# 0xC0000054/avif-format

Measured on NVIDIA H100. Metric: Gpixels/s, higher is better.
Workload: dtype f32

## Files before the change

### avif-format_b200/csrc/avifgpu_api.cu

```cuda
#include "../../include/avifgpu.h"

#include "batch_plan.h"
#include "curve_tables.h"
#include "host_params.h"
#include "kernel_params.h"

#include <cuda_runtime.h>

#include <algorithm>
#include <atomic>
#include <condition_variable>
#include <cstdio>
#include <cstdlib>
#include <cstring>
#include <mutex>
#include <new>
#include <string>
#include <thread>
#include <vector>


namespace avifgpu
{
namespace
{
    thread_local int g_launchFailure = 0;
}

int ReportLaunchFailure(int cudaErrorCode)
{
    g_launchFailure = cudaErrorCode;
    return AVIFGPU_ERR_CUDA;
}

static int TakeLaunchFailure()
{
    const int code = g_launchFailure;
    g_launchFailure = 0;
    return code;
}

int LaunchEncode(const EncodeParams& params, int hostDepth, void* stream)
{
    const EncodeFamily family = EncodeFamilyOf(params, hostDepth);
    const Interior inner = EncodeBlockInterior(family, params, hostDepth);
    if (inner.width == 0)
    {
        return LaunchEncodeGeneric(params, hostDepth, stream);
    }
    cudaError_t e;
    switch (family)
    {
    case EncodeFamily::RgbF32Interleaved: e = LaunchEncodeRgbF32Interleaved(params, inner, stream); break;
    case EncodeFamily::Gray16Lut: e = LaunchEncodeGray16Lut(params, inner, stream); break;
    case EncodeFamily::GrayInt: e = LaunchEncodeGrayInt(params, hostDepth, inner, stream); break;
    case EncodeFamily::RgbInt: e = LaunchEncodeRgbInt(params, hostDepth, inner, stream); break;
    case EncodeFamily::GrayF32: e = LaunchEncodeGrayF32(params, inner, stream); break;
    default: e = LaunchEncodeRgbF32Planar(family, params, inner, stream); break;
    }
    return CompleteEncode(e, params, hostDepth, inner.width, inner.rows, stream);
}

// ... 282 lines not shown
    void FirstUseEncode(const avifgpu_encode_desc& d, int64_t pixels, bool capturing, EncodeParams* p)
    {
        if (CurveTable* table = CurveTableFor(d, pixels, false, capturing))
        {
            p->curveTable = table->valid ? &table->view : nullptr;
        }
        p->gray16Lut = Gray16LutFor(d, capturing);
        p->verifiedPremultiply = VerifiedPremultiply(d, capturing);
    }

    void FirstUseDecode(const avifgpu_decode_desc& d, int32_t transfer, bool capturing, DecodeParams* p)
    {
        p->verifiedHlgDivisions = (d.host_depth == 32 && transfer == AVIFGPU_TRANSFER_HLG) ? VerifiedHlgDivisions(capturing) : 0;
        p->verifiedGreenDivision = VerifiedGreenDivision(*p, capturing);
        p->verifiedPqRatio = (d.host_depth == 32 && transfer == AVIFGPU_TRANSFER_PQ && d.colorspace == AVIFGPU_COLORSPACE_YCBCR) ? VerifiedPqRatio(capturing) : 0;
    }

    int Fail(int status, const std::string& message)
    {
        lastError = message;
        return status;
    }

    int LaunchFailed(int status, const char* what, bool capturing = false)
    {
        const int code = TakeLaunchFailure();
        for (const Slot& slot : slots)
        {
            if (slot.stream && !capturing)
            {
                cudaStreamSynchronize(slot.stream);
            }
        }
        cudaGetLastError();
        lastError = std::string(what) + " failed: " + (code != 0 ? cudaGetErrorString(static_cast<cudaError_t>(code)) : avifgpu_status_string(status));
        return status;
    }

    int Cuda(cudaError_t e, const char* what)
    {
        if (e == cudaSuccess)
        {
            return AVIFGPU_OK;
        }
        lastError = std::string(what) + ": " + cudaGetErrorString(e);
        return (e == cudaErrorMemoryAllocation) ? AVIFGPU_ERR_OOM : AVIFGPU_ERR_CUDA;
// ... 170 lines not shown
    }
    avifgpu_context* ctx = new (std::nothrow) avifgpu_context();
    if (ctx == nullptr)
    {
        g_creationError = "out of host memory";
        return AVIFGPU_ERR_OOM;
    }
    ctx->device = device_ordinal;
    ctx->smCount = prop.multiProcessorCount;
    DeviceGuard guard(device_ordinal);
    for (int i = 0; i < kPipelineStreams; ++i)
    {
        avifgpu_context::Slot& slot = ctx->slots[i];
        if (cudaStreamCreateWithFlags(&slot.stream, cudaStreamNonBlocking) != cudaSuccess ||
            cudaEventCreateWithFlags(&slot.sliceDone, cudaEventDisableTiming) != cudaSuccess ||
            cudaEventCreateWithFlags(&slot.rowsConsumed, cudaEventDisableTiming) != cudaSuccess ||
            (i < 2 && cudaEventCreateWithFlags(&ctx->callRowsConsumed[i], cudaEventDisableTiming) != cudaSuccess))
        {
            g_creationError = std::string("stream/event creation failed: ") + cudaGetErrorString(cudaGetLastError());
            avifgpu_destroy(ctx);
            return AVIFGPU_ERR_CUDA;
        }
    }
    *out_ctx = ctx;
    return AVIFGPU_OK;
}

AVIFGPU_EXPORT void avifgpu_destroy(avifgpu_context* ctx)
{
    if (ctx == nullptr)
    {
        return;
    }
    DeviceGuard guard(ctx->device);
    cudaDeviceSynchronize();
    for (int i = 0; i < kPipelineStreams; ++i)
    {
        const avifgpu_context::Slot& slot = ctx->slots[i];
        if (slot.stream) cudaStreamDestroy(slot.stream);
        if (slot.sliceDone) cudaEventDestroy(slot.sliceDone);
        if (slot.rowsConsumed) cudaEventDestroy(slot.rowsConsumed);
        if (i < 2 && ctx->callRowsConsumed[i]) cudaEventDestroy(ctx->callRowsConsumed[i]);
        for (int b = 0; b < kSlotBuffers; ++b)
        {
            if (slot.device[b].ptr) cudaFree(slot.device[b].ptr);
            if (slot.pinned[b].ptr) cudaFreeHost(slot.pinned[b].ptr);
        }
    }
    for (auto& b : ctx->transferScratch)
    {
        if (b.ptr) cudaFree(b.ptr);
    }
    for (CurveTable* t : ctx->curveTables)
    {
        FreeCurveTable(t);
        delete t;
    }
    for (auto& l : ctx->gray16Luts)
    {
        cudaFree(l.device);
    }
    delete ctx;
}

AVIFGPU_EXPORT const char* avifgpu_last_error(const avifgpu_context* ctx)
{
    return ctx ? ctx->lastError.c_str() : g_creationError.c_str();
}

AVIFGPU_EXPORT int64_t avifgpu_launch_count(const avifgpu_context* ctx) { return ctx ? ctx->launches : 0; }

AVIFGPU_EXPORT int avifgpu_synchronize(avifgpu_context* ctx)
{
    if (ctx == nullptr)
    {
// ... 152 lines not shown
    p.rowCount = nrows;
    for (int k = 0; k < AVIFGPU_MAX_PLANES; ++k)
    {
        const PlaneGeometry g = EncodePlaneGeometry(*desc, k);
        if (!g.present)
        {
            continue;
        }
        if (device_dst->data[k] == nullptr)
        {
            return ctx->Fail(AVIFGPU_ERR_BAD_PARAM, "missing destination plane");
        }
        p.plane[k] = static_cast<uint8_t*>(device_dst->data[k]) + static_cast<int64_t>(y0 >> g.ys) * device_dst->stride[k];
        p.planeStride[k] = device_dst->stride[k];
    }
    DeviceGuard guard(ctx->device);
    bool capturing;
    if ((status = QueryCapture(ctx, cuda_stream, &capturing)) != AVIFGPU_OK)
    {
        return status;
    }
    p.smCount = ctx->smCount;
    ctx->FirstUseEncode(*desc, static_cast<int64_t>(desc->width) * nrows, capturing, &p);
    const int launched = LaunchEncode(p, desc->host_depth, cuda_stream);
    if (launched < 0)
    {
        return ctx->LaunchFailed(launched, "encode kernel launch", capturing);
    }
    ctx->launches += launched;
    return AVIFGPU_OK;
}

AVIFGPU_EXPORT int avifgpu_decode_rows_device(avifgpu_context* ctx, const avifgpu_decode_desc* desc,
                                              const avifgpu_planes* device_src, int32_t y0, int32_t nrows, void* device_rows,
                                              int64_t row_stride_bytes, void* cuda_stream)
{
    if (ctx == nullptr)
    {
        return AVIFGPU_ERR_BAD_PARAM;
    }
    avifgpu_decode_desc full;
    desc = WidenDecodeDesc(desc, &full);
    std::string error;
    int32_t transfer;
    int status = ValidateDecodeDesc(desc, &transfer, &error);
    if (status != AVIFGPU_OK)
    {
// ... 102 lines not shown
    bool capturing;
    int status = QueryCapture(ctx, cuda_stream, &capturing);
    if (status != AVIFGPU_OK)
    {
        return status;
    }
    shared.smCount = ctx->smCount;
    ctx->FirstUseEncode(*desc, pixels, capturing, &shared);
    BatchPlan plan;
    PlanEncodeBatch(shared, desc->host_depth, planeMask, images, count, &plan);
    for (const BatchChunk& chunk : plan.chunks)
    {
        const int launched = LaunchEncodeBatchChunk(shared, desc->host_depth, chunk, cuda_stream);
        if (launched < 0)
        {
            return ctx->LaunchFailed(launched, "batched encode kernel launch", capturing);
        }
        ctx->launches += launched;
    }
    for (const int32_t i : plan.fallback)
    {
        EncodeParams p = shared;
        AdoptBatchImage(p, planeMask, images[i]);
        const int launched = LaunchEncode(p, desc->host_depth, cuda_stream);
        if (launched < 0)
        {
            return ctx->LaunchFailed(launched, "encode kernel launch", capturing);
        }
        ctx->launches += launched;
    }
    return AVIFGPU_OK;
}

AVIFGPU_EXPORT int avifgpu_decode_batch_device(avifgpu_context* ctx, const avifgpu_decode_desc* desc, const avifgpu_batch_image* images,
                                               int32_t count, void* cuda_stream)
{
    if (ctx == nullptr)
    {
        return AVIFGPU_ERR_BAD_PARAM;
    }
    if (desc == nullptr || count < 0 || (count > 0 && images == nullptr))
    {
        return ctx->Fail(AVIFGPU_ERR_BAD_PARAM, "NULL description or image array");
    }
    avifgpu_decode_desc full;
    desc = WidenDecodeDesc(desc, &full);
    avifgpu_decode_desc d = *desc;
// ... 664 lines not shown
            (status = ctx->Cuda(cudaEventRecord(slot.rowsConsumed, slot.stream), "cudaEventRecord")) != AVIFGPU_OK) return AbandonCall(ctx, status);
        callSlots[index] = true;
        if (!wait && rowsPinned && begin + sliceRows >= nrows)
        {
            for (int s = 0; s < kPipelineStreams; ++s)
            {
                if (s != index && callSlots[s] &&
                    (status = ctx->Cuda(cudaStreamWaitEvent(slot.stream, ctx->slots[s].rowsConsumed, 0), "cudaStreamWaitEvent")) != AVIFGPU_OK) return AbandonCall(ctx, status);
            }
            if ((status = ctx->Cuda(cudaEventRecord(ctx->callRowsConsumed[ctx->asyncEncodeCalls & 1], slot.stream), "cudaEventRecord")) != AVIFGPU_OK) return AbandonCall(ctx, status);
            recordedCallRows = true;
        }

        if ((status = EnsureDeviceStaging(ctx, slot, out, planes)) != AVIFGPU_OK) return AbandonCall(ctx, status);
        EncodeParams p = base;
        p.rows = slot.device[kRowsBuffer].ptr;
        p.rowStride = deviceRowStride;
        p.rowCount = rows;
        for (int i = 0; i < planes; ++i)
        {
            p.plane[out[i].buffer] = slot.device[out[i].buffer].ptr;
            p.planeStride[out[i].buffer] = out[i].deviceStride;
        }
        const int launched = LaunchEncode(p, desc->host_depth, slot.stream);
        if (launched < 0)
        {
            return AbandonCall(ctx, ctx->LaunchFailed(launched, "encode kernel launch"));
        }
        ctx->launches += launched;

        if ((status = StageOut(ctx, slot, out, planes)) != AVIFGPU_OK || (status = CloseSlice(ctx, slot, ticket)) != AVIFGPU_OK) return AbandonCall(ctx, status);
    }
    status = FinishCall(ctx, previousRows, ticket, wait);
    if (status == AVIFGPU_OK && !wait && recordedCallRows)
    {
        ctx->asyncEncodeCalls += 1;
        ctx->previousCallRowsPending = true;
    }
    return status;
}

static int DecodeRowsHost(avifgpu_context* ctx, const avifgpu_decode_desc* desc, const avifgpu_planes* src, int32_t y0, int32_t nrows,
                          void* host_rows, int64_t row_stride_bytes, bool wait, int64_t* out_ticket)
{
    if (ctx == nullptr)
    {
        return AVIFGPU_ERR_BAD_PARAM;
// ... 599 lines not shown
```

### avif-format_b200/csrc/kernel_params.h

```cpp
#ifndef AVIF_KERNEL_PARAMS_H
#define AVIF_KERNEL_PARAMS_H

#include <stddef.h>
#include <stdint.h>

#include <atomic>
#include <vector>

#include <driver_types.h>

#include "../../include/avifgpu.h"
#include "curve_tables.h"
#include "pixel_math.cuh"

#if defined(__CUDACC__)
#define AVIFGPU_HD __host__ __device__
#else
#define AVIFGPU_HD
#endif

namespace avifgpu
{

#if defined(__CUDACC__)
// ... 52 lines not shown
    uint32_t maxCode;
    float maxCodeFloat;
    int32_t transfer;
    float pqMultiplier;
    int32_t gray16Smpte428;
    int32_t planar;
    int32_t xs, ys;
    int32_t topLeft;
    avifpix::ForwardMatrix matrix;
    float chromaOffset;
    int32_t hlgInverseOotf;
    float hlgLuma[3];
    float hlgDisplayGamma;
    float hlgPeak;
    int32_t rowMatrixEnabled;
    float rowMatrix[9];
    CurveTableView curveView;
    int32_t useCurveView;
    const CurveTableView* curveTable;
    const uint16_t* gray16Lut;
    int32_t smCount;
    int32_t verifiedPremultiply;
    int32_t destLayout;
};

struct DecodeParams
{
    const void* plane[4];
    int64_t planeStride[4];
    void* rows;
    int64_t rowStride;
    int32_t width;
    int32_t rowCount;
    int32_t yPhase;
    int32_t colorspace;
    int32_t xs, ys;
    int32_t hasAlpha;
    int32_t premultiplied;
    int32_t bitDepth;
    uint32_t maxCode;
    avifpix::RangeParams range;
    avifpix::InverseMatrix matrix;
    int32_t hostDepth;
    int32_t transfer;
    float pqMultiplier;
    int32_t applyOotf;
// ... 477 lines not shown
```

### avif-format_b200/csrc/kernels_fast.cu

```cuda
#include "kernels_fast_common.cuh"
#include "launch_keys.h"
#include "../../include/avifgpu.h"

#include <cuda_runtime.h>

namespace avifgpu
{

using namespace avifpix;
using namespace fastenc;
using avifmath::LibmTables;

namespace
{

constexpr int kClipThreads = 256;
constexpr int kClipWarps = kClipThreads / 32;
constexpr int kClipBlocksPerSm = 3;

template <int XS, int YS, int DEST>
__device__ __forceinline__ void EncodeRgbF32ClipBody(const FastEncodeParams& p)
{
    const int lane = threadIdx.x & 31;
    const int warpInBlock = threadIdx.x >> 5;
// ... 95 lines not shown
    else
    {
        EncodeDestRgbF32ClipKernel<XS, YS, DEST><<<grid, kClipThreads, 0, stream>>>(fp);
    }
    return cudaGetLastError();
}

}

cudaError_t LaunchEncodeRgbF32Interleaved(const EncodeParams& p, Interior inner, void* streamHandle)
{
    FastEncodeParams fp{};
    fp.rows = static_cast<const uint8_t*>(p.rows);
    fp.rowStride = p.rowStride;
    fp.planeY = static_cast<uint8_t*>(p.plane[0]);
    fp.strideY = p.planeStride[0];
    fp.width = inner.width;
    fp.rowCount = inner.rows;
    fp.pqMultiplier = p.pqMultiplier;
    fp.maxCodeFloat = p.maxCodeFloat;
    fp.maxCode = static_cast<int32_t>(p.maxCode);
    fp.table = *p.curveTable;
    const int curve = p.transfer == AVIFGPU_TRANSFER_PQ ? kCurveLinearToPQ : kCurveLinearToSMPTE428;
    return LaunchFastEncodeFlatInterleaved(fp, curve, SmCountOrDefault(p.smCount), static_cast<cudaStream_t>(streamHandle));
}

cudaError_t LaunchEncodeRgbF32Planar(EncodeFamily family, const EncodeParams& p, Interior inner, void* streamHandle)
{
    cudaStream_t stream = static_cast<cudaStream_t>(streamHandle);
    const int curve = p.transfer == AVIFGPU_TRANSFER_PQ ? kCurveLinearToPQ : p.transfer == AVIFGPU_TRANSFER_SMPTE428 ? kCurveLinearToSMPTE428 : kCurveClip;
    FastEncodeParams fp{};
    fp.rows = static_cast<const uint8_t*>(p.rows);
    fp.rowStride = p.rowStride;
    fp.planeY = static_cast<uint8_t*>(p.plane[0]);
    fp.strideY = p.planeStride[0];
    fp.planeCb = static_cast<uint8_t*>(p.plane[1]);
    fp.strideCb = p.planeStride[1];
    fp.planeCr = static_cast<uint8_t*>(p.plane[2]);
    fp.strideCr = p.planeStride[2];
    fp.width = inner.width;
    fp.rowCount = inner.rows;
    fp.pqMultiplier = p.pqMultiplier;
    fp.maxCodeFloat = p.maxCodeFloat;
    fp.maxCode = static_cast<int32_t>(p.maxCode);
    fp.matrix = p.matrix;
    fp.chromaOffset = p.chromaOffset;
    fp.topLeft = p.topLeft;
    if (family != EncodeFamily::RgbF32Clip)
    {
        fp.table = *p.curveTable;
    }
    const int smCount = SmCountOrDefault(p.smCount);
    switch (family)
    {
    case EncodeFamily::RgbaF32Flat:
        fp.planeA = static_cast<uint8_t*>(p.plane[3]);
        fp.strideA = p.planeStride[3];
        fp.premultiply = p.premultiply;
        return LaunchFastEncodeRgba(fp, curve, p.xs, p.ys, p.destLayout, smCount, stream);
    case EncodeFamily::RgbF32Flat: return LaunchFastEncodeFlat(fp, curve, p.xs, p.ys, p.destLayout, smCount, stream);
    default:
        return WithChroma(p.xs, p.ys, [&](auto xs, auto ys) {
            return WithLayout(p.destLayout, [&](auto dest) { return LaunchClipKernel<xs(), ys(), dest()>(fp, smCount, stream); });
        });
    }
}

}
```

### avif-format_b200/csrc/kernels_fast_common.cuh

```cuda
#ifndef AVIF_KERNELS_FAST_COMMON_CUH
#define AVIF_KERNELS_FAST_COMMON_CUH

#include "kernel_params.h"
#include "curve_lookup.cuh"
#include "packed_f32x2.cuh"
#include "source_units.cuh"

#include <cuda_runtime.h>

namespace avifgpu
{
namespace fastenc
{

using namespace avifpix;

constexpr int kTilePixels = 128;
constexpr int kValuesPerLane = 24;
constexpr int kCurveClip = 2;

struct FastEncodeParams
{
    const uint8_t* rows;
    int64_t rowStride;
// ... 163 lines not shown
            }
            StoreChromaWords<DEST>(p, cbRow + r * p.strideCb, crRow + r * p.strideCr, cbWord, crWord);
        }
    }
    else
    {
#pragma unroll
        for (int r = 0; r < 2; ++r)
        {
            if (r == 1 && !secondRow) break;
            const uint32_t cbEven = quantisePair(addOffset(cb2[r][0])), cbOdd = quantisePair(addOffset(cb2[r][1]));
            const uint32_t crEven = quantisePair(addOffset(cr2[r][0])), crOdd = quantisePair(addOffset(cr2[r][1]));
            StoreChromaWords<DEST>(p, cbRow + r * p.strideCb, crRow + r * p.strideCr,
                                   make_uint2(__byte_perm(cbEven, cbOdd, 0x5410), __byte_perm(cbEven, cbOdd, 0x7632)),
                                   make_uint2(__byte_perm(crEven, crOdd, 0x5410), __byte_perm(crEven, crOdd, 0x7632)));
        }
    }
}

}

cudaError_t LaunchFastEncodeRgba(const fastenc::FastEncodeParams& fp, int curve, int xs, int ys, int dest, int smCount, cudaStream_t stream);

cudaError_t LaunchFastEncodeFlat(const fastenc::FastEncodeParams& fp, int curve, int xs, int ys, int dest, int smCount, cudaStream_t stream);
cudaError_t LaunchFastEncodeFlatInterleaved(const fastenc::FastEncodeParams& fp, int curve, int smCount, cudaStream_t stream);

}

#endif
```

### avif-format_b200/csrc/kernels_fast_flat.cu

```cuda
#include "kernels_fast_common.cuh"
#include "launch_keys.h"
#include "table_staging.cuh"
#include "../../include/avifgpu.h"

namespace avifgpu
{

using namespace avifpix;
using namespace fastenc;
using namespace staging;
using avifmath::LibmTables;

namespace
{

constexpr int kFlatThreads = kFlatWarps * 32;
constexpr int kRowSegmentBytes = kTilePixels * 12;
static_assert(kFlatStageBytesPerWarp == 2 * kRowSegmentBytes, "a warp's staging buffer holds both rows of its tile");
constexpr int kRowSegmentWords = kRowSegmentBytes / 4;
constexpr int kTableBarrierSlot = kFlatSharedBarriers / 8 - 1;
static_assert(kFlatWarps <= kTableBarrierSlot, "the warps' barriers and the table's share kFlatSharedBarriers");

struct FlatSchedule
{
    int32_t tilesX, tileRows, warpCount;
    int32_t segments, items;
    int32_t segmentRows, longSegments;
    int32_t lastColumnBytes;
    int32_t unpairedTileRow;
};

__device__ __forceinline__ bool ElectOne()
{
    uint32_t elected;
    asm volatile("{ .reg .pred p; elect.sync _|p, 0xffffffff; selp.u32 %0, 1, 0, p; }" : "=r"(elected));
    return elected != 0;
}

constexpr int kTableTwoLevel = 1;
constexpr int kTableCompact = 2;
constexpr int kTableCompact14 = 3;

template <int CURVE, int XS, int YS, int TABLE, int INTERLEAVED, int DEST>
__device__ __forceinline__ void EncodeRgbF32FlatBody(const FastEncodeParams& p, const FlatSchedule& schedule)
{
    constexpr bool kCompact = TABLE != kTableTwoLevel;
    constexpr int kCompactShift = TABLE == kTableCompact14 ? 14 : 0;
    extern __shared__ __align__(128) uint8_t sharedBytes[];
    uint64_t* libmStorage = reinterpret_cast<uint64_t*>(sharedBytes);
    uint64_t* barriers = reinterpret_cast<uint64_t*>(sharedBytes + kSharedLibm);
    uint8_t* stageAll = sharedBytes + kSharedLibm + kFlatSharedBarriers;
    uint32_t* compactEntries = reinterpret_cast<uint32_t*>(sharedBytes + FlatFixedBytes());
    const uint32_t* firstBits = compactEntries + ((p.table.flatCount + 3) & ~3);
    uint2* octaves = reinterpret_cast<uint2*>(sharedBytes + FlatFixedBytes());
    uint32_t* bucketWords = reinterpret_cast<uint32_t*>(sharedBytes + FlatFixedBytes() + kFlatOctaveBytes);

    const int lane = threadIdx.x & 31;
    const int warpInBlock = __shfl_sync(0xffffffffu, static_cast<int>(threadIdx.x >> 5), 0);
    const uint32_t barrier = SharedAddress(barriers + warpInBlock);
    uint32_t* stage = reinterpret_cast<uint32_t*>(stageAll + warpInBlock * kFlatStageBytesPerWarp);
    const uint32_t stageAddress = SharedAddress(stage);
    const uint32_t* myStage = stage + lane * 12;

    const int tilesX = schedule.tilesX;
    const int warpCount = schedule.warpCount;
    const int firstItem = warpInBlock * static_cast<int>(gridDim.x) + static_cast<int>(blockIdx.x);
    constexpr int kChromaRowsPerTile = YS ? 1 : 2;
    constexpr int kChromaPairs = SourceInterleaved(DEST) ? 2 : 1;
    constexpr int kChromaTileBytes = (XS ? kTilePixels : 2 * kTilePixels) * kChromaPairs;

    auto itemRows = [&](int item, int& column, int& rowBegin, int& rowEnd)
    {
        const int segment = item / tilesX;
        column = item - segment * tilesX;
        rowBegin = segment * schedule.segmentRows + min(segment, schedule.longSegments);
        rowEnd = rowBegin + schedule.segmentRows + (segment < schedule.longSegments ? 1 : 0);
    };
    auto fetchTile = [&](int row, uint32_t bytes, int64_t offset)
    {
        const bool second = row != schedule.unpairedTileRow;
        const uint8_t* source = p.rows + offset;
        BarrierExpect(barrier, second ? 2u * bytes : bytes);
        BulkCopyToShared(stageAddress, source, bytes, barrier);
        if (second)
        {
            BulkCopyToShared(stageAddress + kRowSegmentBytes, source + p.rowStride, bytes, barrier);
        }
    };
    auto columnBytes = [&](int column) { return column == tilesX - 1 ? static_cast<uint32_t>(schedule.lastColumnBytes) : static_cast<uint32_t>(kRowSegmentBytes); };
    auto sourceOffsetOf = [&](int row, int column) { return static_cast<int64_t>(row) * 2 * p.rowStride + static_cast<int64_t>(column) * kRowSegmentBytes; };

    if (kCompact && threadIdx.x == 0)
    {
        BeginTableImageCopy(p.table, compactEntries, barriers + kTableBarrierSlot);
    }
    if (ElectOne())
    {
        BarrierInit(barrier, 1);
        BarrierInitFence();
        if (firstItem < schedule.items)
        {
            int column, rowBegin, rowEnd;
            itemRows(firstItem, column, rowBegin, rowEnd);
            if (rowBegin < rowEnd)
            {
                fetchTile(rowBegin, columnBytes(column), sourceOffsetOf(rowBegin, column));
            }
        }
    }

    const LibmTables t = avifmath::StageLibmTables(libmStorage, threadIdx.x, blockDim.x);
    if (!kCompact)
    {
        for (int i = threadIdx.x; i < 256; i += blockDim.x)
        {
            octaves[i] = p.table.octaves[i];
        }
        for (int i = threadIdx.x; i < p.table.bucketCount; i += blockDim.x)
        {
            bucketWords[i] = p.table.buckets[i];
        }
    }
    __syncthreads();
    if (kCompact)
    {
        WaitTableImage(barriers + kTableBarrierSlot);
    }

    const uint32_t flatShift = p.table.flatShift;
    const int32_t negativeLow = -static_cast<int32_t>(p.table.flatLow);
    const int32_t span = static_cast<int32_t>(p.table.flatHigh - p.table.flatLow);
    const uint32_t bandStrideLog2 = p.table.bandStrideLog2;
    const uint32_t* __restrict__ bandBits = p.table.bandBits;
    const uint32_t compactTopShift = 32u - flatShift;
    const uint32_t compactCodeMask = p.table.compactCodeMask;
    const uint32_t compactMagic = p.table.compactMagic;
    uint32_t parity = 0;

#pragma unroll 1
    for (int item = firstItem; item < schedule.items; item += warpCount)
    {
        int column, rowBegin, rowEnd;
        itemRows(item, column, rowBegin, rowEnd);
        if (item != firstItem && rowBegin < rowEnd && ElectOne())
        {
            fetchTile(rowBegin, columnBytes(column), sourceOffsetOf(rowBegin, column));
        }
        const uint32_t tileBytes = columnBytes(column);
        const bool laneActive = column * kTilePixels + lane * 4 < p.width;
        int64_t sourceOffset = sourceOffsetOf(rowBegin, column);
        uint8_t* yPointer = p.planeY + static_cast<int64_t>(rowBegin) * 2 * p.strideY +
                            (INTERLEAVED ? static_cast<int64_t>(column) * (6 * kTilePixels) + lane * 24 : static_cast<int64_t>(column) * (2 * kTilePixels) + lane * 8);
        uint8_t* cbPointer = p.planeCb + static_cast<int64_t>(rowBegin) * kChromaRowsPerTile * p.strideCb + static_cast<int64_t>(column) * kChromaTileBytes + lane * (XS ? 4 : 8) * kChromaPairs;
        uint8_t* crPointer = p.planeCr + static_cast<int64_t>(rowBegin) * kChromaRowsPerTile * p.strideCr + static_cast<int64_t>(column) * kChromaTileBytes + lane * (XS ? 4 : 8);

#pragma unroll 1
    for (int tileRow = rowBegin; tileRow < rowEnd; ++tileRow)
    {
        const bool secondRow = tileRow != schedule.unpairedTileRow;
        sourceOffset += 2 * p.rowStride;

        BarrierWait(barrier, parity);
        parity ^= 1u;

        float codeF[kValuesPerLane];
        uint32_t bandMask = 0;
        int32_t largest = 0;
#pragma unroll
        for (int q = 0; q < 6; ++q)
        {
            const uint4 w = *reinterpret_cast<const uint4*>(myStage + (q / 3) * kRowSegmentWords + (q % 3) * 4);
            const uint32_t bits[4] = { w.x, w.y, w.z, w.w };
#pragma unroll
            for (int e = 0; e < 4; ++e)
            {
                const int j = 4 * q + e;
                bool inBand;
                if (kCompact)
                {
                    uint32_t entry;
                    codeF[j] = LookupCurveCompact<kCompactShift>(bits[e], compactEntries, flatShift, negativeLow, span, compactTopShift, compactCodeMask,
                                                                 compactMagic, inBand, entry);
                }
// ... 50 lines not shown
        }

        if (__any_sync(0xffffffffu, kCompact ? largest > 0x7f7fffff : bandMask != 0))
        {
            for (int j = 0; j < kValuesPerLane; ++j)
            {
                const uint32_t bits = stagedBits(j);
                if (kCompact ? static_cast<int32_t>(bits) > 0x7f7fffff : ((bandMask >> j) & 1u) != 0)
                {
                    const float exact = CodeToFloat(ExactCurveCode<CURVE>(__uint_as_float(bits), p.pqMultiplier, p.maxCodeFloat, t));
#pragma unroll
                    for (int slot = 0; slot < kValuesPerLane; ++slot)
                    {
                        if (slot == j)
                        {
                            codeF[slot] = exact;
                        }
                    }
                }
            }
        }

        __syncwarp();
        if (tileRow + 1 < rowEnd && ElectOne())
        {
            fetchTile(tileRow + 1, tileBytes, sourceOffset);
        }

#pragma unroll
        for (int j = 0; j < kValuesPerLane; ++j)
        {
            if (lowerMask & (1u << j))
            {
                codeF[j] -= 1.0f;
            }
        }

        if (laneActive)
        {
            if (INTERLEAVED)
            {
#pragma unroll
                for (int r = 0; r < 2; ++r)
                {
                    if (r == 1 && !secondRow) break;
                    uint32_t words[6];
#pragma unroll
                    for (int w = 0; w < 6; ++w)
                    {
                        words[w] = __float2uint_rz(codeF[12 * r + 2 * w]) | (__float2uint_rz(codeF[12 * r + 2 * w + 1]) << 16);
                    }
                    uint2* target = reinterpret_cast<uint2*>(yPointer + r * p.strideY);
                    __stcs(target, make_uint2(words[0], words[1]));
                    __stcs(target + 1, make_uint2(words[2], words[3]));
                    __stcs(target + 2, make_uint2(words[4], words[5]));
                }
            }
            else
            {
                StoreTile<XS, YS, DEST>(p, codeF, yPointer, cbPointer, crPointer, secondRow);
            }
        }
        yPointer += 2 * p.strideY;
        cbPointer += kChromaRowsPerTile * p.strideCb;
        crPointer += kChromaRowsPerTile * p.strideCr;
    }
    }
}

template <int CURVE, int XS, int YS, int TABLE, int INTERLEAVED>
__global__ void __launch_bounds__(kFlatThreads, 1) EncodeRgbF32FlatKernel(const FastEncodeParams p, const FlatSchedule schedule)
{
    EncodeRgbF32FlatBody<CURVE, XS, YS, TABLE, INTERLEAVED, AVIFGPU_SOURCE_PLANAR>(p, schedule);
}

template <int CURVE, int XS, int YS, int TABLE, int DEST>
__global__ void __launch_bounds__(kFlatThreads, 1) EncodeDestRgbF32FlatKernel(const FastEncodeParams p, const FlatSchedule schedule)
{
    EncodeRgbF32FlatBody<CURVE, XS, YS, TABLE, 0, DEST>(p, schedule);
}

template <int CURVE, int XS, int YS, int TABLE, int INTERLEAVED, int DEST>
constexpr auto FlatKernelFor()
{
    if constexpr (DEST == AVIFGPU_SOURCE_PLANAR)
    {
        return EncodeRgbF32FlatKernel<CURVE, XS, YS, TABLE, INTERLEAVED>;
    }
    else
    {
        return EncodeDestRgbF32FlatKernel<CURVE, XS, YS, TABLE, DEST>;
    }
}

template <int CURVE, int XS, int YS, int TABLE, int INTERLEAVED = 0, int DEST = AVIFGPU_SOURCE_PLANAR>
cudaError_t LaunchFlatKernel(const FastEncodeParams& fp, int smCount, cudaStream_t stream)
{
    const size_t shared = static_cast<size_t>(FlatFixedBytes()) + FlatTableBytes(fp.table, TABLE == kTableTwoLevel);
    static std::atomic<uint64_t> configuredDevices{ 0 };
    {
        const cudaError_t e = AllowDynamicShared(FlatKernelFor<CURVE, XS, YS, TABLE, INTERLEAVED, DEST>(), kSharedLimit, configuredDevices);
        if (e != cudaSuccess)
        {
            return e;
        }
    }
    const long long tiles = static_cast<long long>((fp.width + kTilePixels - 1) / kTilePixels) * ((fp.rowCount + 1) / 2);
    if (tiles > 0x7fffffffll || shared > static_cast<size_t>(kSharedLimit))
    {
        return cudaErrorInvalidValue;
    }
    long long blocks = (tiles + kFlatWarps - 1) / kFlatWarps;
    if (blocks > smCount)
    {
        blocks = smCount;
    }
    FlatSchedule schedule{};
    schedule.tilesX = (fp.width + kTilePixels - 1) / kTilePixels;
    schedule.tileRows = (fp.rowCount + 1) / 2;
    schedule.warpCount = static_cast<int32_t>(blocks) * kFlatWarps;
    schedule.segments = schedule.warpCount / schedule.tilesX;
    if (schedule.segments < 1) schedule.segments = 1;
    if (schedule.segments > schedule.tileRows) schedule.segments = schedule.tileRows;
    schedule.items = schedule.tilesX * schedule.segments;
    schedule.segmentRows = schedule.tileRows / schedule.segments;
    schedule.longSegments = schedule.tileRows % schedule.segments;
    schedule.lastColumnBytes = (fp.width - (schedule.tilesX - 1) * kTilePixels) * 12;
    schedule.unpairedTileRow = (fp.rowCount & 1) ? fp.rowCount / 2 : -1;
    FlatKernelFor<CURVE, XS, YS, TABLE, INTERLEAVED, DEST>()<<<static_cast<unsigned>(blocks), kFlatThreads, shared, stream>>>(fp, schedule);
    return cudaGetLastError();
}

}

cudaError_t LaunchFastEncodeFlatInterleaved(const FastEncodeParams& fp, int curve, int smCount, cudaStream_t stream)
{
    if (FlatCompactFits(fp.table))
    {
        if (curve == kCurveLinearToPQ)
        {
            return fp.table.flatShift == 14 ? LaunchFlatKernel<kCurveLinearToPQ, 0, 0, kTableCompact14, 1>(fp, smCount, stream)
                                            : LaunchFlatKernel<kCurveLinearToPQ, 0, 0, kTableCompact, 1>(fp, smCount, stream);
        }
        return LaunchFlatKernel<kCurveLinearToSMPTE428, 0, 0, kTableCompact, 1>(fp, smCount, stream);
    }
    if (curve == kCurveLinearToPQ) return LaunchFlatKernel<kCurveLinearToPQ, 0, 0, kTableTwoLevel, 1>(fp, smCount, stream);
    return LaunchFlatKernel<kCurveLinearToSMPTE428, 0, 0, kTableTwoLevel, 1>(fp, smCount, stream);
}

cudaError_t LaunchFastEncodeFlat(const FastEncodeParams& fp, int curve, int xs, int ys, int dest, int smCount, cudaStream_t stream)
{
    return WithChroma(xs, ys, [&](auto XS, auto YS) {
        return WithLayout(dest, [&](auto DEST) {
            if (FlatCompactFits(fp.table))
            {
                if (curve == kCurveLinearToPQ)
                {
                    return fp.table.flatShift == 14 ? LaunchFlatKernel<kCurveLinearToPQ, XS(), YS(), kTableCompact14, 0, DEST()>(fp, smCount, stream)
                                                    : LaunchFlatKernel<kCurveLinearToPQ, XS(), YS(), kTableCompact, 0, DEST()>(fp, smCount, stream);
                }
                return LaunchFlatKernel<kCurveLinearToSMPTE428, XS(), YS(), kTableCompact, 0, DEST()>(fp, smCount, stream);
            }
            if constexpr (DEST() == AVIFGPU_SOURCE_PLANAR)
            {
                if (curve == kCurveLinearToPQ) return LaunchFlatKernel<kCurveLinearToPQ, XS(), YS(), kTableTwoLevel>(fp, smCount, stream);
            }
            else if (curve == kCurveLinearToPQ)
            {
                return cudaErrorInvalidValue;
            }
            return LaunchFlatKernel<kCurveLinearToSMPTE428, XS(), YS(), kTableTwoLevel, 0, DEST()>(fp, smCount, stream);
        });
    });
}

}
```

Baseline: 178.7.

## Add dynamic tile stealing tail to flat encode kernel schedule

The flat RGB f32 encode kernel now gives each warp a static share covering about 90% of the tile rows. The remaining tail is handed out dynamically through a global atomic tile counter in runs of two tile rows. The host keeps a pool of device counters guarded by events so that concurrent launches do not share one, and the last grabbing warp resets its counter to zero. The aim is to even out load imbalance between warps at the end of the frame, at the cost of atomics, extra host bookkeeping and event queries per launch.

```diff
diff --git a/avif-format_b200/csrc/avifgpu_api.cu b/avif-format_b200/csrc/avifgpu_api.cu
--- a/avif-format_b200/csrc/avifgpu_api.cu
+++ b/avif-format_b200/csrc/avifgpu_api.cu
@@ -38,6 +38,13 @@
     const int code = g_launchFailure;
     g_launchFailure = 0;
     return code;
+}
+
+static bool UsesFlatKernel(const EncodeParams& params, int hostDepth)
+{
+    const EncodeFamily family = EncodeFamilyOf(params, hostDepth);
+    return (family == EncodeFamily::RgbF32Flat || family == EncodeFamily::RgbF32Interleaved) &&
+           EncodeBlockInterior(family, params, hostDepth).width != 0;
 }
 
 int LaunchEncode(const EncodeParams& params, int hostDepth, void* stream)
@@ -366,6 +373,97 @@
         return status;
     }
 
+    struct TileCounter
+    {
+        uint32_t* device = nullptr;
+        cudaEvent_t done = nullptr;
+        bool pending = false;
+        bool captured = false;
+    };
+    static constexpr int kTileCountersPerBlock = 64;
+    std::vector<TileCounter> tileCounters;
+    std::vector<uint32_t*> tileCounterBlocks;
+    size_t nextTileCounter = 0;
+
+    int GrowTileCounters(cudaStream_t stream)
+    {
+        uint32_t* block = nullptr;
+        int status = Cuda(cudaMalloc(&block, kTileCountersPerBlock * sizeof(uint32_t)), "cudaMalloc");
+        if (status != AVIFGPU_OK)
+        {
+            return status;
+        }
+        tileCounterBlocks.push_back(block);
+        if ((status = Cuda(cudaMemsetAsync(block, 0, kTileCountersPerBlock * sizeof(uint32_t), stream), "cudaMemsetAsync")) != AVIFGPU_OK)
+        {
+            return status;
+        }
+        for (int i = 0; i < kTileCountersPerBlock; ++i)
+        {
+            TileCounter c;
+            c.device = block + i;
+            if ((status = Cuda(cudaEventCreateWithFlags(&c.done, cudaEventDisableTiming), "cudaEventCreateWithFlags")) != AVIFGPU_OK)
+            {
+                return status;
+            }
+            tileCounters.push_back(c);
+            if ((status = Cuda(cudaEventRecord(c.done, stream), "cudaEventRecord")) != AVIFGPU_OK)
+            {
+                tileCounters.back().captured = true;
+                return status;
+            }
+            tileCounters.back().pending = true;
+        }
+        return AVIFGPU_OK;
+    }
+
+    int TakeTileCounter(cudaStream_t stream, bool capturing)
+    {
+        const size_t n = tileCounters.size();
+        for (size_t k = 0; k < n; ++k)
+        {
+            const size_t i = (nextTileCounter + k) % n;
+            TileCounter& c = tileCounters[i];
+            if (c.captured || (c.pending && (capturing || cudaEventQuery(c.done) != cudaSuccess)))
+            {
+                continue;
+            }
+            c.pending = false;
+            nextTileCounter = (i + 1) % n;
+            return static_cast<int>(i);
+        }
+        if (capturing || GrowTileCounters(stream) != AVIFGPU_OK)
+        {
+            cudaGetLastError();
+            return -1;
+        }
+        nextTileCounter = n + 1;
+        tileCounters[n].pending = false;
+        return static_cast<int>(n);
+    }
+
+    int LaunchEncodeCounted(EncodeParams p, int hostDepth, void* stream, bool capturing)
+    {
+        const cudaStream_t s = static_cast<cudaStream_t>(stream);
+        const int counter = UsesFlatKernel(p, hostDepth) ? TakeTileCounter(s, capturing) : -1;
+        p.tileCounter = counter >= 0 ? tileCounters[counter].device : nullptr;
+        const int launched = LaunchEncode(p, hostDepth, stream);
+        if (launched >= 0 && counter >= 0)
+        {
+            TileCounter& c = tileCounters[counter];
+            if (capturing || cudaEventRecord(c.done, s) != cudaSuccess)
+            {
+                c.captured = true;
+                cudaGetLastError();
+            }
+            else
+            {
+                c.pending = true;
+            }
+        }
+        return launched;
+    }
+
     int LaunchFailed(int status, const char* what, bool capturing = false)
     {
         const int code = TakeLaunchFailure();
@@ -582,6 +680,13 @@
             return AVIFGPU_ERR_CUDA;
         }
     }
+    if (ctx->GrowTileCounters(ctx->slots[0].stream) != AVIFGPU_OK || cudaStreamSynchronize(ctx->slots[0].stream) != cudaSuccess)
+    {
+        g_creationError = "tile counter allocation failed: " + ctx->lastError;
+        cudaGetLastError();
+        avifgpu_destroy(ctx);
+        return AVIFGPU_ERR_CUDA;
+    }
     *out_ctx = ctx;
     return AVIFGPU_OK;
 }
@@ -611,6 +716,14 @@
     {
         if (b.ptr) cudaFree(b.ptr);
     }
+    for (const auto& c : ctx->tileCounters)
+    {
+        cudaEventDestroy(c.done);
+    }
+    for (uint32_t* block : ctx->tileCounterBlocks)
+    {
+        cudaFree(block);
+    }
     for (CurveTable* t : ctx->curveTables)
     {
         FreeCurveTable(t);
@@ -809,7 +922,7 @@
     }
     p.smCount = ctx->smCount;
     ctx->FirstUseEncode(*desc, static_cast<int64_t>(desc->width) * nrows, capturing, &p);
-    const int launched = LaunchEncode(p, desc->host_depth, cuda_stream);
+    const int launched = ctx->LaunchEncodeCounted(p, desc->host_depth, cuda_stream, capturing);
     if (launched < 0)
     {
         return ctx->LaunchFailed(launched, "encode kernel launch", capturing);
@@ -958,7 +1071,7 @@
     {
         EncodeParams p = shared;
         AdoptBatchImage(p, planeMask, images[i]);
-        const int launched = LaunchEncode(p, desc->host_depth, cuda_stream);
+        const int launched = ctx->LaunchEncodeCounted(p, desc->host_depth, cuda_stream, capturing);
         if (launched < 0)
         {
             return ctx->LaunchFailed(launched, "encode kernel launch", capturing);
@@ -1669,7 +1782,7 @@
             p.plane[out[i].buffer] = slot.device[out[i].buffer].ptr;
             p.planeStride[out[i].buffer] = out[i].deviceStride;
         }
-        const int launched = LaunchEncode(p, desc->host_depth, slot.stream);
+        const int launched = ctx->LaunchEncodeCounted(p, desc->host_depth, slot.stream, false);
         if (launched < 0)
         {
             return AbandonCall(ctx, ctx->LaunchFailed(launched, "encode kernel launch"));
diff --git a/avif-format_b200/csrc/flat_schedule.h b/avif-format_b200/csrc/flat_schedule.h
--- /dev/null
+++ b/avif-format_b200/csrc/flat_schedule.h
@@ -0,0 +1,72 @@
+#ifndef AVIF_FLAT_SCHEDULE_H
+#define AVIF_FLAT_SCHEDULE_H
+
+#include "kernel_params.h"
+
+namespace avifgpu
+{
+
+constexpr int kFlatTileWidth = 128;
+constexpr int kFlatStaticPercent = 90;
+constexpr int kFlatGrabRows = 2;
+
+struct FlatSchedule
+{
+    int32_t tilesX, tileRows, warpCount;
+    int32_t segments, items;
+    int32_t segmentRows, longSegments;
+    int32_t staticRows;
+    uint32_t grabRuns;
+    int32_t lastColumnBytes;
+    int32_t unpairedTileRow;
+    uint32_t* tileCounter;
+};
+
+inline FlatSchedule MakeFlatSchedule(int width, int rowCount, int smCount, uint32_t* tileCounter)
+{
+    FlatSchedule s{};
+    s.tilesX = (width + kFlatTileWidth - 1) / kFlatTileWidth;
+    s.tileRows = (rowCount + 1) / 2;
+    const long long blocks = (static_cast<long long>(s.tilesX) * s.tileRows + kFlatWarps - 1) / kFlatWarps;
+    s.warpCount = static_cast<int32_t>(blocks < smCount ? blocks : smCount) * kFlatWarps;
+    s.segments = s.warpCount / s.tilesX;
+    if (s.segments < 1) s.segments = 1;
+    if (s.segments > s.tileRows) s.segments = s.tileRows;
+    if (tileCounter == nullptr)
+    {
+        s.staticRows = s.tileRows;
+        s.segmentRows = s.tileRows / s.segments;
+        s.longSegments = s.tileRows % s.segments;
+    }
+    else
+    {
+        s.segmentRows = static_cast<int32_t>(static_cast<int64_t>(s.tileRows) * kFlatStaticPercent / 100 / s.segments);
+        s.staticRows = s.segments * s.segmentRows;
+    }
+    s.items = s.staticRows > 0 ? s.tilesX * s.segments : 0;
+    s.grabRuns = static_cast<uint32_t>(s.tilesX) * static_cast<uint32_t>((s.tileRows - s.staticRows + kFlatGrabRows - 1) / kFlatGrabRows);
+    s.lastColumnBytes = (width - (s.tilesX - 1) * kFlatTileWidth) * 12;
+    s.unpairedTileRow = (rowCount & 1) ? rowCount / 2 : -1;
+    s.tileCounter = tileCounter;
+    return s;
+}
+
+AVIFGPU_HD inline void FlatItemRows(const FlatSchedule& s, int item, int& column, int& rowBegin, int& rowEnd)
+{
+    const int segment = item / s.tilesX;
+    column = item - segment * s.tilesX;
+    rowBegin = segment * s.segmentRows + (segment < s.longSegments ? segment : s.longSegments);
+    rowEnd = rowBegin + s.segmentRows + (segment < s.longSegments ? 1 : 0);
+}
+
+AVIFGPU_HD inline void FlatGrabRun(const FlatSchedule& s, uint32_t index, int& row, int& column, int& runEnd)
+{
+    const uint32_t band = index / static_cast<uint32_t>(s.tilesX);
+    row = s.staticRows + static_cast<int>(band) * kFlatGrabRows;
+    column = static_cast<int>(index - band * static_cast<uint32_t>(s.tilesX));
+    runEnd = row + kFlatGrabRows < s.tileRows ? row + kFlatGrabRows : s.tileRows;
+}
+
+}
+
+#endif
diff --git a/avif-format_b200/csrc/kernel_params.h b/avif-format_b200/csrc/kernel_params.h
--- a/avif-format_b200/csrc/kernel_params.h
+++ b/avif-format_b200/csrc/kernel_params.h
@@ -98,6 +98,7 @@
     int32_t smCount;
     int32_t verifiedPremultiply;
     int32_t destLayout;
+    uint32_t* tileCounter;
 };
 
 struct DecodeParams
diff --git a/avif-format_b200/csrc/kernels_fast.cu b/avif-format_b200/csrc/kernels_fast.cu
--- a/avif-format_b200/csrc/kernels_fast.cu
+++ b/avif-format_b200/csrc/kernels_fast.cu
@@ -141,7 +141,7 @@
     fp.maxCode = static_cast<int32_t>(p.maxCode);
     fp.table = *p.curveTable;
     const int curve = p.transfer == AVIFGPU_TRANSFER_PQ ? kCurveLinearToPQ : kCurveLinearToSMPTE428;
-    return LaunchFastEncodeFlatInterleaved(fp, curve, SmCountOrDefault(p.smCount), static_cast<cudaStream_t>(streamHandle));
+    return LaunchFastEncodeFlatInterleaved(fp, curve, SmCountOrDefault(p.smCount), p.tileCounter, static_cast<cudaStream_t>(streamHandle));
 }
 
 cudaError_t LaunchEncodeRgbF32Planar(EncodeFamily family, const EncodeParams& p, Interior inner, void* streamHandle)
@@ -177,7 +177,7 @@
         fp.strideA = p.planeStride[3];
         fp.premultiply = p.premultiply;
         return LaunchFastEncodeRgba(fp, curve, p.xs, p.ys, p.destLayout, smCount, stream);
-    case EncodeFamily::RgbF32Flat: return LaunchFastEncodeFlat(fp, curve, p.xs, p.ys, p.destLayout, smCount, stream);
+    case EncodeFamily::RgbF32Flat: return LaunchFastEncodeFlat(fp, curve, p.xs, p.ys, p.destLayout, smCount, p.tileCounter, stream);
     default:
         return WithChroma(p.xs, p.ys, [&](auto xs, auto ys) {
             return WithLayout(p.destLayout, [&](auto dest) { return LaunchClipKernel<xs(), ys(), dest()>(fp, smCount, stream); });
diff --git a/avif-format_b200/csrc/kernels_fast_common.cuh b/avif-format_b200/csrc/kernels_fast_common.cuh
--- a/avif-format_b200/csrc/kernels_fast_common.cuh
+++ b/avif-format_b200/csrc/kernels_fast_common.cuh
@@ -209,8 +209,9 @@
 
 cudaError_t LaunchFastEncodeRgba(const fastenc::FastEncodeParams& fp, int curve, int xs, int ys, int dest, int smCount, cudaStream_t stream);
 
-cudaError_t LaunchFastEncodeFlat(const fastenc::FastEncodeParams& fp, int curve, int xs, int ys, int dest, int smCount, cudaStream_t stream);
-cudaError_t LaunchFastEncodeFlatInterleaved(const fastenc::FastEncodeParams& fp, int curve, int smCount, cudaStream_t stream);
+cudaError_t LaunchFastEncodeFlat(const fastenc::FastEncodeParams& fp, int curve, int xs, int ys, int dest, int smCount, uint32_t* tileCounter,
+                                 cudaStream_t stream);
+cudaError_t LaunchFastEncodeFlatInterleaved(const fastenc::FastEncodeParams& fp, int curve, int smCount, uint32_t* tileCounter, cudaStream_t stream);
 
 }
 
diff --git a/avif-format_b200/csrc/kernels_fast_flat.cu b/avif-format_b200/csrc/kernels_fast_flat.cu
--- a/avif-format_b200/csrc/kernels_fast_flat.cu
+++ b/avif-format_b200/csrc/kernels_fast_flat.cu
@@ -1,4 +1,5 @@
 #include "kernels_fast_common.cuh"
+#include "flat_schedule.h"
 #include "launch_keys.h"
 #include "table_staging.cuh"
 #include "../../include/avifgpu.h"
@@ -21,14 +22,7 @@
 constexpr int kTableBarrierSlot = kFlatSharedBarriers / 8 - 1;
 static_assert(kFlatWarps <= kTableBarrierSlot, "the warps' barriers and the table's share kFlatSharedBarriers");
 
-struct FlatSchedule
-{
-    int32_t tilesX, tileRows, warpCount;
-    int32_t segments, items;
-    int32_t segmentRows, longSegments;
-    int32_t lastColumnBytes;
-    int32_t unpairedTileRow;
-};
+static_assert(kFlatTileWidth == kTilePixels, "flat_schedule.h deals the kernel's tiles");
 
 __device__ __forceinline__ bool ElectOne()
 {
@@ -69,13 +63,6 @@
     constexpr int kChromaPairs = SourceInterleaved(DEST) ? 2 : 1;
     constexpr int kChromaTileBytes = (XS ? kTilePixels : 2 * kTilePixels) * kChromaPairs;
 
-    auto itemRows = [&](int item, int& column, int& rowBegin, int& rowEnd)
-    {
-        const int segment = item / tilesX;
-        column = item - segment * tilesX;
-        rowBegin = segment * schedule.segmentRows + min(segment, schedule.longSegments);
-        rowEnd = rowBegin + schedule.segmentRows + (segment < schedule.longSegments ? 1 : 0);
-    };
     auto fetchTile = [&](int row, uint32_t bytes, int64_t offset)
     {
         const bool second = row != schedule.unpairedTileRow;
@@ -90,23 +77,60 @@
     auto columnBytes = [&](int column) { return column == tilesX - 1 ? static_cast<uint32_t>(schedule.lastColumnBytes) : static_cast<uint32_t>(kRowSegmentBytes); };
     auto sourceOffsetOf = [&](int row, int column) { return static_cast<int64_t>(row) * 2 * p.rowStride + static_cast<int64_t>(column) * kRowSegmentBytes; };
 
+    uint32_t* const tileCounter = schedule.tileCounter;
+    int item = firstItem - warpCount;
+    uint32_t grab = 0;
+    auto grabsAfter = [&](int row, int runEnd) { return tileCounter != nullptr && row + 1 == runEnd && item + warpCount >= schedule.items; };
+    auto nextRun = [&](int& row, int& column, int& runEnd)
+    {
+        if (item < schedule.items)
+        {
+            item += warpCount;
+            if (item < schedule.items)
+            {
+                FlatItemRows(schedule, item, column, row, runEnd);
+                return true;
+            }
+        }
+        if (tileCounter == nullptr)
+        {
+            return false;
+        }
+        const uint32_t index = __shfl_sync(0xffffffffu, grab, 0);
+        if (lane == 0 && index == schedule.grabRuns + static_cast<uint32_t>(warpCount) - 1u)
+        {
+            atomicExch(tileCounter, 0u);
+        }
+        if (index >= schedule.grabRuns)
+        {
+            return false;
+        }
+        FlatGrabRun(schedule, index, row, column, runEnd);
+        return true;
+    };
+
     if (kCompact && threadIdx.x == 0)
     {
         BeginTableImageCopy(p.table, compactEntries, barriers + kTableBarrierSlot);
     }
+    if (tileCounter != nullptr && firstItem >= schedule.items && lane == 0)
+    {
+        grab = atomicAdd(tileCounter, 1u);
+    }
+    int row, column, runEnd;
+    bool more = nextRun(row, column, runEnd);
     if (ElectOne())
     {
         BarrierInit(barrier, 1);
         BarrierInitFence();
-        if (firstItem < schedule.items)
-        {
-            int column, rowBegin, rowEnd;
-            itemRows(firstItem, column, rowBegin, rowEnd);
-            if (rowBegin < rowEnd)
-            {
-                fetchTile(rowBegin, columnBytes(column), sourceOffsetOf(rowBegin, column));
-            }
-        }
+        if (more)
+        {
+            fetchTile(row, columnBytes(column), sourceOffsetOf(row, column));
+        }
+    }
+    if (more && lane == 0 && grabsAfter(row, runEnd))
+    {
+        grab = atomicAdd(tileCounter, 1u);
     }
 
     const LibmTables t = avifmath::StageLibmTables(libmStorage, threadIdx.x, blockDim.x);
@@ -137,28 +161,24 @@
     const uint32_t compactMagic = p.table.compactMagic;
     uint32_t parity = 0;
 
+    uint8_t* yPointer;
+    uint8_t* cbPointer;
+    uint8_t* crPointer;
+    bool laneActive;
+    auto pointTo = [&](int row, int column)
+    {
+        laneActive = column * kTilePixels + lane * 4 < p.width;
+        yPointer = p.planeY + static_cast<int64_t>(row) * 2 * p.strideY +
+                   (INTERLEAVED ? static_cast<int64_t>(column) * (6 * kTilePixels) + lane * 24 : static_cast<int64_t>(column) * (2 * kTilePixels) + lane * 8);
+        cbPointer = p.planeCb + static_cast<int64_t>(row) * kChromaRowsPerTile * p.strideCb + static_cast<int64_t>(column) * kChromaTileBytes + lane * (XS ? 4 : 8) * kChromaPairs;
+        crPointer = p.planeCr + static_cast<int64_t>(row) * kChromaRowsPerTile * p.strideCr + static_cast<int64_t>(column) * kChromaTileBytes + lane * (XS ? 4 : 8);
+    };
+    pointTo(row, column);
+
 #pragma unroll 1
-    for (int item = firstItem; item < schedule.items; item += warpCount)
-    {
-        int column, rowBegin, rowEnd;
-        itemRows(item, column, rowBegin, rowEnd);
-        if (item != firstItem && rowBegin < rowEnd && ElectOne())
-        {
-            fetchTile(rowBegin, columnBytes(column), sourceOffsetOf(rowBegin, column));
-        }
-        const uint32_t tileBytes = columnBytes(column);
-        const bool laneActive = column * kTilePixels + lane * 4 < p.width;
-        int64_t sourceOffset = sourceOffsetOf(rowBegin, column);
-        uint8_t* yPointer = p.planeY + static_cast<int64_t>(rowBegin) * 2 * p.strideY +
-                            (INTERLEAVED ? static_cast<int64_t>(column) * (6 * kTilePixels) + lane * 24 : static_cast<int64_t>(column) * (2 * kTilePixels) + lane * 8);
-        uint8_t* cbPointer = p.planeCb + static_cast<int64_t>(rowBegin) * kChromaRowsPerTile * p.strideCb + static_cast<int64_t>(column) * kChromaTileBytes + lane * (XS ? 4 : 8) * kChromaPairs;
-        uint8_t* crPointer = p.planeCr + static_cast<int64_t>(rowBegin) * kChromaRowsPerTile * p.strideCr + static_cast<int64_t>(column) * kChromaTileBytes + lane * (XS ? 4 : 8);
-
-#pragma unroll 1
-    for (int tileRow = rowBegin; tileRow < rowEnd; ++tileRow)
-    {
-        const bool secondRow = tileRow != schedule.unpairedTileRow;
-        sourceOffset += 2 * p.rowStride;
+    while (more)
+    {
+        const bool secondRow = row != schedule.unpairedTileRow;
 
         BarrierWait(barrier, parity);
         parity ^= 1u;
@@ -255,9 +275,16 @@
         }
 
         __syncwarp();
-        if (tileRow + 1 < rowEnd && ElectOne())
-        {
-            fetchTile(tileRow + 1, tileBytes, sourceOffset);
+        int nextRow = row + 1, nextColumn = column, nextRunEnd = runEnd;
+        const bool sameRun = nextRow < runEnd;
+        more = sameRun || nextRun(nextRow, nextColumn, nextRunEnd);
+        if (more && ElectOne())
+        {
+            fetchTile(nextRow, columnBytes(nextColumn), sourceOffsetOf(nextRow, nextColumn));
+        }
+        if (more && lane == 0 && grabsAfter(nextRow, nextRunEnd))
+        {
+            grab = atomicAdd(tileCounter, 1u);
         }
 
 #pragma unroll
@@ -294,10 +321,19 @@
                 StoreTile<XS, YS, DEST>(p, codeF, yPointer, cbPointer, crPointer, secondRow);
             }
         }
-        yPointer += 2 * p.strideY;
-        cbPointer += kChromaRowsPerTile * p.strideCb;
-        crPointer += kChromaRowsPerTile * p.strideCr;
-    }
+        if (sameRun)
+        {
+            yPointer += 2 * p.strideY;
+            cbPointer += kChromaRowsPerTile * p.strideCb;
+            crPointer += kChromaRowsPerTile * p.strideCr;
+        }
+        else
+        {
+            pointTo(nextRow, nextColumn);
+        }
+        row = nextRow;
+        column = nextColumn;
+        runEnd = nextRunEnd;
     }
 }
 
@@ -327,7 +363,7 @@
 }
 
 template <int CURVE, int XS, int YS, int TABLE, int INTERLEAVED = 0, int DEST = AVIFGPU_SOURCE_PLANAR>
-cudaError_t LaunchFlatKernel(const FastEncodeParams& fp, int smCount, cudaStream_t stream)
+cudaError_t LaunchFlatKernel(const FastEncodeParams& fp, int smCount, uint32_t* tileCounter, cudaStream_t stream)
 {
     const size_t shared = static_cast<size_t>(FlatFixedBytes()) + FlatTableBytes(fp.table, TABLE == kTableTwoLevel);
     static std::atomic<uint64_t> configuredDevices{ 0 };
@@ -343,45 +379,29 @@
     {
         return cudaErrorInvalidValue;
     }
-    long long blocks = (tiles + kFlatWarps - 1) / kFlatWarps;
-    if (blocks > smCount)
-    {
-        blocks = smCount;
-    }
-    FlatSchedule schedule{};
-    schedule.tilesX = (fp.width + kTilePixels - 1) / kTilePixels;
-    schedule.tileRows = (fp.rowCount + 1) / 2;
-    schedule.warpCount = static_cast<int32_t>(blocks) * kFlatWarps;
-    schedule.segments = schedule.warpCount / schedule.tilesX;
-    if (schedule.segments < 1) schedule.segments = 1;
-    if (schedule.segments > schedule.tileRows) schedule.segments = schedule.tileRows;
-    schedule.items = schedule.tilesX * schedule.segments;
-    schedule.segmentRows = schedule.tileRows / schedule.segments;
-    schedule.longSegments = schedule.tileRows % schedule.segments;
-    schedule.lastColumnBytes = (fp.width - (schedule.tilesX - 1) * kTilePixels) * 12;
-    schedule.unpairedTileRow = (fp.rowCount & 1) ? fp.rowCount / 2 : -1;
-    FlatKernelFor<CURVE, XS, YS, TABLE, INTERLEAVED, DEST>()<<<static_cast<unsigned>(blocks), kFlatThreads, shared, stream>>>(fp, schedule);
+    const FlatSchedule schedule = MakeFlatSchedule(fp.width, fp.rowCount, smCount, tileCounter);
+    FlatKernelFor<CURVE, XS, YS, TABLE, INTERLEAVED, DEST>()<<<static_cast<unsigned>(schedule.warpCount / kFlatWarps), kFlatThreads, shared, stream>>>(fp, schedule);
     return cudaGetLastError();
 }
 
 }
 
-cudaError_t LaunchFastEncodeFlatInterleaved(const FastEncodeParams& fp, int curve, int smCount, cudaStream_t stream)
+cudaError_t LaunchFastEncodeFlatInterleaved(const FastEncodeParams& fp, int curve, int smCount, uint32_t* tileCounter, cudaStream_t stream)
 {
     if (FlatCompactFits(fp.table))
     {
         if (curve == kCurveLinearToPQ)
         {
-            return fp.table.flatShift == 14 ? LaunchFlatKernel<kCurveLinearToPQ, 0, 0, kTableCompact14, 1>(fp, smCount, stream)
-                                            : LaunchFlatKernel<kCurveLinearToPQ, 0, 0, kTableCompact, 1>(fp, smCount, stream);
-        }
-        return LaunchFlatKernel<kCurveLinearToSMPTE428, 0, 0, kTableCompact, 1>(fp, smCount, stream);
-    }
-    if (curve == kCurveLinearToPQ) return LaunchFlatKernel<kCurveLinearToPQ, 0, 0, kTableTwoLevel, 1>(fp, smCount, stream);
-    return LaunchFlatKernel<kCurveLinearToSMPTE428, 0, 0, kTableTwoLevel, 1>(fp, smCount, stream);
-}
-
-cudaError_t LaunchFastEncodeFlat(const FastEncodeParams& fp, int curve, int xs, int ys, int dest, int smCount, cudaStream_t stream)
+            return fp.table.flatShift == 14 ? LaunchFlatKernel<kCurveLinearToPQ, 0, 0, kTableCompact14, 1>(fp, smCount, tileCounter, stream)
+                                            : LaunchFlatKernel<kCurveLinearToPQ, 0, 0, kTableCompact, 1>(fp, smCount, tileCounter, stream);
+        }
+        return LaunchFlatKernel<kCurveLinearToSMPTE428, 0, 0, kTableCompact, 1>(fp, smCount, tileCounter, stream);
+    }
+    if (curve == kCurveLinearToPQ) return LaunchFlatKernel<kCurveLinearToPQ, 0, 0, kTableTwoLevel, 1>(fp, smCount, tileCounter, stream);
+    return LaunchFlatKernel<kCurveLinearToSMPTE428, 0, 0, kTableTwoLevel, 1>(fp, smCount, tileCounter, stream);
+}
+
+cudaError_t LaunchFastEncodeFlat(const FastEncodeParams& fp, int curve, int xs, int ys, int dest, int smCount, uint32_t* tileCounter, cudaStream_t stream)
 {
     return WithChroma(xs, ys, [&](auto XS, auto YS) {
         return WithLayout(dest, [&](auto DEST) {
@@ -389,20 +409,20 @@
             {
                 if (curve == kCurveLinearToPQ)
                 {
-                    return fp.table.flatShift == 14 ? LaunchFlatKernel<kCurveLinearToPQ, XS(), YS(), kTableCompact14, 0, DEST()>(fp, smCount, stream)
-                                                    : LaunchFlatKernel<kCurveLinearToPQ, XS(), YS(), kTableCompact, 0, DEST()>(fp, smCount, stream);
-                }
-                return LaunchFlatKernel<kCurveLinearToSMPTE428, XS(), YS(), kTableCompact, 0, DEST()>(fp, smCount, stream);
+                    return fp.table.flatShift == 14 ? LaunchFlatKernel<kCurveLinearToPQ, XS(), YS(), kTableCompact14, 0, DEST()>(fp, smCount, tileCounter, stream)
+                                                    : LaunchFlatKernel<kCurveLinearToPQ, XS(), YS(), kTableCompact, 0, DEST()>(fp, smCount, tileCounter, stream);
+                }
+                return LaunchFlatKernel<kCurveLinearToSMPTE428, XS(), YS(), kTableCompact, 0, DEST()>(fp, smCount, tileCounter, stream);
             }
             if constexpr (DEST() == AVIFGPU_SOURCE_PLANAR)
             {
-                if (curve == kCurveLinearToPQ) return LaunchFlatKernel<kCurveLinearToPQ, XS(), YS(), kTableTwoLevel>(fp, smCount, stream);
+                if (curve == kCurveLinearToPQ) return LaunchFlatKernel<kCurveLinearToPQ, XS(), YS(), kTableTwoLevel>(fp, smCount, tileCounter, stream);
             }
             else if (curve == kCurveLinearToPQ)
             {
                 return cudaErrorInvalidValue;
             }
-            return LaunchFlatKernel<kCurveLinearToSMPTE428, XS(), YS(), kTableTwoLevel, 0, DEST()>(fp, smCount, stream);
+            return LaunchFlatKernel<kCurveLinearToSMPTE428, XS(), YS(), kTableTwoLevel, 0, DEST()>(fp, smCount, tileCounter, stream);
         });
     });
 }
diff --git a/profiles/measure_flat_frame.py b/profiles/measure_flat_frame.py
--- /dev/null
+++ b/profiles/measure_flat_frame.py
@@ -0,0 +1,84 @@
+#!/usr/bin/env python3
+import statistics
+
+import harness
+import torch
+
+import avifgpu
+import bench
+from harness import timed
+
+HEIGHTS = (1080, 2160, 4320, 8640)
+L2_BYTES = 50 * 2**20
+
+
+def frame_way(ctx, height, sets):
+    wl = bench.Workload("c2", rows=height)
+    assert wl.pixels * 12 > L2_BYTES, "every input set must be larger than L2"
+    inputs = [wl.make_device_input(torch, torch.device("cuda", 0), 2000 + 17 * i)[0] for i in range(sets)]
+    outputs = [avifgpu.planes_from_tensors(wl.make_device_output(torch, torch.device("cuda", 0))) for _ in range(sets)]
+    turn = [0]
+
+    def run():
+        i = turn[0] % sets
+        turn[0] += 1
+        rows = inputs[i]
+        ctx.encode_device(wl.enc, rows.data_ptr(), rows.stride(0) * rows.element_size(), outputs[i])
+
+    return run, wl.algorithmic_bytes
+
+
+def fit(points):
+    xs, ys = [x for x, _ in points], [y for _, y in points]
+    mx, my = statistics.mean(xs), statistics.mean(ys)
+    slope = sum((x - mx) * (y - my) for x, y in points) / sum((x - mx) ** 2 for x in xs)
+    return my - slope * mx, slope
+
+
+def bounds(seconds, rounds):
+    n = 2**28
+    a = torch.rand(n, device="cuda")
+    b = torch.empty_like(a)
+    total = torch.empty((), device="cuda")
+    ms = timed({"copy": lambda: b.copy_(a), "sum": lambda: torch.sum(a, 0, out=total)}, seconds, rounds)
+    size = n * 4
+    return {"d2d_copy_gbs": 2 * size / (statistics.median(ms["copy"]) * 1e-3) / 1e9,
+            "read_sum_gbs": size / (statistics.median(ms["sum"]) * 1e-3) / 1e9,
+            "note": "torch.Tensor.copy_ counts read + write bytes, torch.sum read bytes; 1 GiB float32 each"}
+
+
+def main():
+    ap = harness.arguments(rounds=5)
+    ap.add_argument("--sets", type=int, default=3, help="rotating input / output sets per size (each larger than L2)")
+    args = ap.parse_args()
+    harness.require_gpu()
+    result = {"card": harness.card(), "unit": "microseconds per launch (device events, median of rounds)", "width": 7680}
+    with avifgpu.Context(0) as ctx:
+        ctx.prepare_encode(bench.Workload("c2").enc)
+        ways, sizes = {}, {}
+        for h in HEIGHTS:
+            ways[h], sizes[h] = frame_way(ctx, h, args.sets)
+        calls = {}
+        ms = timed(ways, args.seconds, args.rounds, calls=calls)
+        launches_before = ctx.launch_count()
+        ways[HEIGHTS[0]]()
+        torch.cuda.synchronize()
+        result["launches_per_frame"] = ctx.launch_count() - launches_before
+        del ways
+    points, sweep = [], {}
+    for h in HEIGHTS:
+        us = statistics.median(ms[h]) * 1e3
+        points.append((sizes[h], us))
+        sweep[str(h)] = {"bytes": sizes[h], "us": us, "spread_us": (max(ms[h]) - min(ms[h])) * 1e3, "calls_per_window": calls[h],
+                         "tbs": sizes[h] / (us * 1e-6) / 1e12}
+    intercept, slope = fit(points)
+    result["sweep"] = sweep
+    result["fit"] = {"intercept_us": intercept, "steady_tbs": 1.0 / slope / 1e6,
+                     "residuals_us": {str(h): us - (intercept + slope * x) for h, (x, us) in zip(HEIGHTS, points)}}
+    torch.cuda.empty_cache()
+    result["bounds"] = bounds(args.seconds, args.rounds)
+    harness.emit([result], args.out)
+
+
+if __name__ == "__main__":
+    main()
```

After: 183.6, median of 6. +2.7%, better.
